# koadman/mauveAligner

Hardware: AMD Instinct MI355X
Metric: aligned Mbp/s (seed+extend+DP) (higher is better)
Workload: dtype u32; 1 GPU; C3: 5 x 5000000 bp synthetic genomes, ~3% divergence, ~50 inversions, seed weight 15, recursive anchoring + gapped DP on; genomes_per_gpu=5, genome_length=5000000, seed_weight=15, parallelism=independent genome sets per GPU (no data-path collective), extend_lcbs=1, max_extension_iters=4

## Files before the change

### mauvealigner_amd/csrc/api.cpp

```cpp
#include "common.hpp"
#include <dlfcn.h>
#include <algorithm>
#include <cstring>

static thread_local std::string g_create_err;

GenomeSet main_genome_set(mauve_ctx *c)
{
    GenomeSet gs;
    gs.buf = &c->genomes; gs.nseq = c->nseq; gs.lens = c->lens; gs.word_off = c->word_off;
    if (c->has_invalid) gs.vmask = &c->base_invalid;
    if (c->has_contigs) gs.cmask = &c->contig_mask;
    if (c->has_invalid || c->has_contigs) gs.mask_off = c->base_mask_off;
    return gs;
}

struct GenomeTails { uint64_t off[MAUVE_MAX_SEQ]; int64_t len[MAUVE_MAX_SEQ]; uint64_t total_words; };
__global__ void genome_tail_fix(uint64_t *__restrict__ words, GenomeTails gt)
{
    const int g = blockIdx.x;
    const int64_t len = gt.len[g];
    const uint64_t data = (uint64_t)((len + 31) / 32);
    uint64_t *w = words + gt.off[g];
    const uint64_t end = (g + 1 == (int)gridDim.x ? gt.total_words + 4 : gt.off[g + 1]) - gt.off[g];
// ... 195 lines not shown
extern "C" {

static hipError_t create_priority_stream(hipStream_t *out)
{
    int least = 0, greatest = 0;
    if (hipDeviceGetStreamPriorityRange(&least, &greatest) != hipSuccess) { (void)hipGetLastError(); return hipStreamCreateWithFlags(out, hipStreamNonBlocking); }
    return hipStreamCreateWithPriority(out, hipStreamNonBlocking, least);
}

int mauve_ctx_create(int device, mauve_ctx **out)
{
    if (!out) return MAUVE_ERR_ARG;
    *out = nullptr;
    int ndev = 0;
    hipError_t e = hipGetDeviceCount(&ndev);
    if (e != hipSuccess || ndev <= 0) {
        g_create_err = std::string("no HIP device available (") + (e != hipSuccess ? hipGetErrorString(e) : "count = 0") +
                       "); libmauve_hip has no CPU fallback";
        return MAUVE_ERR_NOGPU;
    }
    if (device < 0 || device >= ndev) { g_create_err = "device index out of range"; return MAUVE_ERR_ARG; }
    mauve_ctx *c = new (std::nothrow) mauve_ctx();
    if (!c) { g_create_err = "out of host memory"; return MAUVE_ERR_ARG; }
    c->device = device;
    if (const char *sp = getenv("MAUVE_SCHEDULE")) {
        const unsigned f = !strcmp(sp, "spin") ? hipDeviceScheduleSpin : !strcmp(sp, "yield") ? hipDeviceScheduleYield : hipDeviceScheduleBlockingSync;
        (void)hipSetDevice(device); (void)hipSetDeviceFlags(f); (void)hipGetLastError();
    }
    if ((e = hipSetDevice(device)) != hipSuccess || (e = hipStreamCreateWithFlags(&c->stream, hipStreamNonBlocking)) != hipSuccess ||
        (e = create_priority_stream(&c->stream2)) != hipSuccess ||
        (e = hipStreamCreateWithFlags(&c->stream_io, hipStreamNonBlocking)) != hipSuccess ||
        (e = hipEventCreateWithFlags(&c->ev_io_fork, hipEventDisableTiming)) != hipSuccess ||
        (e = hipEventCreateWithFlags(&c->ev_io_done, hipEventDisableTiming)) != hipSuccess ||
        (e = hipEventCreateWithFlags(&c->ev_fork, hipEventDisableTiming)) != hipSuccess ||
        (e = hipEventCreateWithFlags(&c->ev_join, hipEventDisableTiming)) != hipSuccess ||
        (e = hipEventCreate(&c->ev0)) != hipSuccess || (e = hipEventCreate(&c->ev1)) != hipSuccess) {
        g_create_err = std::string("HIP init failed: ") + hipGetErrorString(e);
        delete c;
        return MAUVE_ERR_HIP;
    }
    hipDeviceProp_t prop;
    if (hipGetDeviceProperties(&prop, device) == hipSuccess) {
        snprintf(c->devname, sizeof c->devname, "%s (%s, %d CUs)", prop.name, prop.gcnArchName, prop.multiProcessorCount);
        if (prop.multiProcessorCount > 0) c->cus = prop.multiProcessorCount;
    }
    c->pool = new (std::nothrow) SpinPool(SpinPool::default_threads());
    if (!c->pool) { g_create_err = "out of host memory"; mauve_ctx_destroy(c); return MAUVE_ERR_ARG; }
    *out = c;
    return MAUVE_OK;
}

void mauve_ctx_destroy(mauve_ctx *c)
{
    if (!c) return;
    (void)hipSetDevice(c->device);
    if (c->stream_io) (void)hipStreamSynchronize(c->stream_io);
    if (c->stream2) (void)hipStreamSynchronize(c->stream2);
    if (c->stream) (void)hipStreamSynchronize(c->stream);
    delete c->pool; c->pool = nullptr;
    DevBuf *bufs[] = {&c->genomes, &c->keysA, &c->keysB, &c->valsA, &c->valsB, &c->hist, &c->totals, &c->posmask,
                      &c->hit_mask, &c->hit_pos, &c->hit_seg, &c->base_invalid, &c->contig_mask, &c->node_cmask, &c->run_sum, &c->join_ovf, &c->join_bound, &c->dpf_anch, &c->dpf_work, &c->dpf_tot, &c->ch_len, &c->ch_st, &c->ch_crop, &c->ch_ent, &c->ch_ord, &c->ch_rank, &c->ch_node, &c->ch_graph, &c->ch_cnt, &c->ch_anch, &c->ch_lw, &c->ch_anch2, &c->ext_work, &c->bp_work, &c->dp_sp, &c->hom_cols, &c->sorted_rec_keep, &c->ch_big, &c->gap_work, &c->as_wide, &c->res_narrow, &c->dp_pick, &c->dp_wflags, &c->ch_mw, &c->shard_dev, &c->as_work, &c->as_isl, &c->res_cols, &c->sorted_rec, &c->canon_k1, &c->canon_k2, &c->canon_v1, &c->canon_v2, &c->rec_genomes, &c->rec_seg, &c->rec_vinv, &c->rec_vcm, &c->placed_mask, &c->bb_cols, &c->bb_work, &c->bb_query, &c->cand, &c->mlen, &c->mstart, &c->counters, &c->dp_desc, &c->dp_list, &c->dp_codes, &c->dp_off,
                      &c->dp_prof_cnt, &c->dp_prof_mask, &c->dp_prof2_cnt, &c->dp_prof2_mask, &c->dp_tb, &c->dp_meta,
                      &c->dp_score, &c->dp_cols, &c->dp_rows, &c->rp_wcnt, &c->rp_mult, &c->pf_mums, &c->co_index, &c->co_q, &c->ex_work, &c->ex_bits, &c->ex_sel, &c->ex_mat, &c->ps_work, &c->ps_out, &c->exc_work, &c->exc_tmp, &c->exc_meta, &c->exc_rec, &c->pj_work, &c->pj_cols, &c->pj_src, &c->pj_out, &c->co_truth_index, &c->sc_out, &c->rm_work, &c->rm_res};
    for (DevBuf *b : bufs) b->release();
    coord_index_release(c);
    c->pin_genomes.release(); c->pin_tail.release(); c->pin_ext.release(); c->pin_chain.release(); c->pin_mask.release(); c->pin_bb.release(); c->pin_asm.release(); c->pin_tab.release(); c->pin_cols.release(); c->pin_anch.release(); c->pin_dcols.release(); c->pin_meta.release(); c->pin_seed.release(); c->pin_dp_in.release(); c->shard_pin.release(); c->pin_stage.release();
    if (c->ev0) (void)hipEventDestroy(c->ev0);
    if (c->ev1) (void)hipEventDestroy(c->ev1);
    if (c->ev_fork) (void)hipEventDestroy(c->ev_fork);
    if (c->ev_join) (void)hipEventDestroy(c->ev_join);
    if (c->ev_io_fork) (void)hipEventDestroy(c->ev_io_fork);
    if (c->ev_io_done) (void)hipEventDestroy(c->ev_io_done);
    if (c->stream_io) (void)hipStreamDestroy(c->stream_io);
    if (c->stream2) (void)hipStreamDestroy(c->stream2);
    if (c->stream) (void)hipStreamDestroy(c->stream);
    delete c;
}

const char *mauve_last_error(const mauve_ctx *c) { return c ? c->err.c_str() : g_create_err.c_str(); }

int mauve_device_name(const mauve_ctx *c, char *buf, size_t buflen)
{
    if (!c || !buf || !buflen) return MAUVE_ERR_ARG;
    snprintf(buf, buflen, "%s", c->devname);
    return MAUVE_OK;
}

int mauve_synchronize(mauve_ctx *c)
{
    if (!c) return MAUVE_ERR_ARG;
    HIPCHK(c, hipStreamSynchronize(c->stream));
    return MAUVE_OK;
}

int mauve_set_shard(mauve_ctx *c, int rank, int world, mauve_allgather_fn fn, void *user)
{
    if (!c) return MAUVE_ERR_ARG;
    c->shard_comm = nullptr; c->shard_stat = mauve_shard_stats{0, 0, 0, 0.0};
    if (world <= 1 || !fn) { c->shard_rank = 0; c->shard_world = 1; c->shard_fn = nullptr; c->shard_user = nullptr; c->shard_on = false; return MAUVE_OK; }
    if (rank < 0 || rank >= world) { c->err = "set_shard: rank outside the world"; return MAUVE_ERR_ARG; }
    c->shard_rank = rank; c->shard_world = world; c->shard_fn = fn; c->shard_user = user; c->shard_on = true;
    return MAUVE_OK;
}

int mauve_set_shard_rccl(mauve_ctx *c, int rank, int world, void *nccl_comm)
// ... 332 lines not shown
```

### mauvealigner_amd/csrc/common.hpp

```cpp
#pragma once
#include <hip/hip_runtime.h>
#include <cstdint>
#include <cstdio>
#include <string>
#include <vector>
#include <functional>
#include "workers.hpp"
#include "host_chain.hpp"
#include "backbone_host.hpp"
#include <chrono>
#include <algorithm>
#include <cstring>

#include "../../include/mauve_hip.h"

#define HIPCHK(ctx, call)                                                                         \
    do {                                                                                          \
        hipError_t e__ = (call);                                                                  \
        if (e__ != hipSuccess) {                                                                  \
            (ctx)->err = std::string(#call) + ": " + hipGetErrorString(e__) + " (" __FILE__ ":" + \
                         std::to_string(__LINE__) + ")";                                          \
            return MAUVE_ERR_HIP;                                                                 \
        }                                                                                         \
    } while (0)
// ... 123 lines not shown
    const int32_t *dv_len = nullptr, *dv_st = nullptr, *dv_lcb = nullptr;
    bool lw_from_host = false;
    int64_t mums_kept = -1;
    mauve_params p{};
    int N = 0; uint32_t full = 0;
    int64_t sum = 0, nm = 0, nl = 0, n_dp = 0, code_total = 0, n_anchor = 0, anchor_cols = 0;
    double t0 = 0, t_dp0 = 0;
    std::vector<MatchVec> chains;
    std::vector<GapRef> gaps;
    std::vector<DpSeqDesc> desc;
    std::vector<int64_t> dcol_off, dscore;
    MatchVec m;
    std::vector<int64_t> match_lcb;
    std::vector<int64_t> match_weight;
    std::vector<Item> items;
    void count_anchors() { for (const MatchVec &ch : chains) { n_anchor += (int64_t)ch.size(); for (size_t i = 0; i < ch.size(); i++) anchor_cols += ch.len(i); } }
    void reset()
    {
        open = false; anchor_table_done = false; dev_tail = false; dv_len = dv_st = dv_lcb = nullptr; lw_from_host = false; mums_kept = -1; p = mauve_params(); N = 0; full = 0;
        sum = nm = nl = n_dp = code_total = n_anchor = anchor_cols = 0; t0 = t_dp0 = 0;
        gaps.clear(); desc.clear(); dcol_off.clear(); dscore.clear();
        match_lcb.clear(); match_weight.clear(); items.clear();
    }
};

struct CoordDev;
struct mauve_ctx {
    int device = 0;
    hipStream_t stream = nullptr;
    hipStream_t stream2 = nullptr;
    hipEvent_t ev_fork = nullptr, ev_join = nullptr;
    hipStream_t stream_io = nullptr;
    hipEvent_t ev_io_fork = nullptr, ev_io_done = nullptr;
    struct TablePrefetch {
        int32_t *mum_length = nullptr, *mum_start = nullptr, *anchor_length = nullptr, *anchor_start = nullptr, *anchor_lcb = nullptr;
        int64_t mum_cap = 0, anchor_cap = 0;
        bool armed = false;
        bool live = false;
        bool inflight = false;
        bool got_mums = false, got_anchors = false;
    } pf;
    DevBuf pf_mums;
    std::string err;
    char devname[256] = {0};
    int cus = 256;

    int nseq = 0;
    std::vector<int64_t> lens;
    std::vector<uint64_t> word_off;
    std::vector<const uint64_t *> host_packed;
    PinnedBuf pin_genomes;
    PinnedBuf pin_tail;
    bool host_copy_valid = false;
    size_t total_words = 0;
    DevBuf genomes;
    DevBuf base_invalid, contig_mask, node_cmask;
    bool has_invalid = false, has_contigs = false;
    std::vector<uint64_t> h_invalid, h_contig, base_mask_off;

    DevBuf keysA, keysB, valsA, valsB, hist, totals, posmask, hit_mask, hit_pos, hit_seg, cand, mlen, mstart, counters;
    DevBuf sorted_rec;
    DevBuf canon_k1, canon_k2, canon_v1, canon_v2;
    DevBuf join_bound;
    DevBuf join_ovf;
    DevBuf ch_len, ch_st, ch_crop, ch_ent, ch_ord, ch_rank, ch_node, ch_graph, ch_cnt;
    DevBuf gap_work;
// ... 157 lines not shown
int refuse_past_2g(mauve_ctx *c, const char *what);
int seedpass_run(mauve_ctx *ctx, const GenomeSet &gs, uint64_t pattern, int mode, uint64_t mask, int extend,
                 const uint32_t *seg_dev, uint32_t nseg, int64_t *n_matches);
int seedpass_enumerate(mauve_ctx *ctx, const GenomeSet &gs, int seq, uint64_t pattern, EnumRequest &q);
int seedpass_from_hits(mauve_ctx *ctx, const GenomeSet &gs, uint64_t pattern, const HostHits &hits, int extend, int64_t *n_matches);
int seedpass_sorted_list(mauve_ctx *ctx, const GenomeSet &gs, int seq, uint64_t pattern, std::vector<uint64_t> *keys,
                         std::vector<uint32_t> *vals, int *weight);

int sort_pairs_u32(mauve_ctx *ctx, uint32_t n, int key_bits, uint32_t **keys_io, uint32_t **vals_io, uint32_t *keys_alt, uint32_t *vals_alt,
                   int timer_id);
int sort_pairs_u32_batch(mauve_ctx *ctx, uint32_t S, uint32_t n, size_t seg_stride, int key_bits, uint32_t **keys_io, uint32_t **vals_io,
                         uint32_t *keys_alt, uint32_t *vals_alt, int timer_id);
int sort_pairs_u64(mauve_ctx *ctx, uint32_t n, int key_bits, uint64_t **keys_io, uint32_t **vals_io, uint64_t *keys_alt, uint32_t *vals_alt,
                   int timer_id);
int seed_finish(mauve_ctx *ctx, const GenomeSet &gs, const SeedRequest &rq, uint32_t ncand, bool on_host, double &trace_t0);
bool seed_trace_on();
uint32_t canon_device_min();
inline void seed_trace(mauve_ctx *ctx, const char *label, double &t0)
{
    if (!seed_trace_on()) return;
    (void)hipStreamSynchronize(ctx->stream);
    const double t = now_ms();
    fprintf(stderr, "[trace] %-22s +%.3f ms\n", label, t - t0);
    t0 = t;
}
inline int seed_counters(mauve_ctx *ctx, size_t bytes, const uint32_t **words)
{
    HIPCHK(ctx, ctx->pin_seed.ensure(64));
    HIPCHK(ctx, hipMemcpyAsync(ctx->pin_seed.p, ctx->counters.p, bytes, hipMemcpyDeviceToHost, ctx->stream));
    HIPCHK(ctx, hipStreamSynchronize(ctx->stream));
    *words = ctx->pin_seed.as<uint32_t>();
    return MAUVE_OK;
}
int chain_device(mauve_ctx *c, int N, int64_t min_weight, bool collinear, MatchVec &m, std::vector<int64_t> &match_lcb, int64_t &n_lcb, const mauve_scoring *sp_scoring = nullptr);
struct ChainGraphHost { uint32_t na, K; int64_t *weight; uint32_t *orient; int32_t *prev, *next; int32_t *final_stage; int32_t *final_dev; };
int chain_device_graph(mauve_ctx *c, int N, int64_t maxlen, const uint32_t *seg0, uint32_t nseg, ChainGraphHost *G, bool graph_to_host = true, const mauve_scoring *sp_scoring = nullptr);
int chain_device_gaps_compact(mauve_ctx *c, int N, int64_t maxlen, const uint32_t *seg0_dev, uint32_t nseg, const int32_t **hl_out, const int32_t **hs_out,
                              const uint32_t **hgap_out, uint32_t *ns_out);
int chain_device_core(mauve_ctx *c, int N, int64_t min_weight, bool collinear, int64_t &n_lcb, const mauve_scoring *sp_scoring = nullptr);
int chain_device_gaps(mauve_ctx *c, int N, int64_t maxlen, const uint32_t *seg0_dev, uint32_t nseg, const int32_t **hl_out, const int32_t **hs_out,
                      std::vector<uint8_t> &survive);
int chain_device_copy_back(mauve_ctx *c, int N, MatchVec &m, std::vector<int64_t> &match_lcb);
int chain_order_device(mauve_ctx *c, int N, int64_t nl, int64_t min_gap, int64_t *na_out, int64_t *n_rec_out);
int extend_lcbs_device(mauve_ctx *c, const mauve_params *p, int w, int64_t lcbw, int N, const int32_t **alen_io, const int32_t **ast_io,
                       const int32_t **alcb_io, int64_t *na_io, int64_t *nl_io, int64_t *n_rec_io, std::vector<int64_t> &lcb_weight);

struct ChainOrders { std::vector<std::vector<uint32_t>> ord; bool sparse = false; };
void host_eliminate_overlaps(MatchVec &m, ChainOrders *orders = nullptr, bool compact = true);
int seed_family_matches(mauve_ctx *c, const GenomeSet &gs, int w, int mode, uint64_t mask, MatchVec &out);
void host_merge_matches(MatchVec &kept, const MatchVec &add);
void host_left_orders(const MatchVec &m, ChainOrders &orders);
void host_lcb_chain(const MatchVec &m, int64_t min_weight, bool collinear, std::vector<int64_t> &match_lcb, int64_t &n_lcb,
                    const ChainOrders *orders = nullptr, const int64_t *match_weight = nullptr);
int match_sp_scores(mauve_ctx *c, const MatchVec &m, const int *gmap, const mauve_scoring *sc, std::vector<int64_t> &out);
int repeat_multiplicity(mauve_ctx *c, uint64_t pattern);
int repeat_matches(mauve_ctx *c, int seq, uint64_t pattern, int64_t min_multi, int64_t max_multi);
int repeat_fetch(mauve_ctx *c, int64_t *length, int64_t *mult, int64_t *start_off, int64_t *starts);
int repeat_begin(mauve_ctx *c, const mauve_params *p, int w, uint64_t pat);
int64_t sp_default_min_weight(int w, int n, const mauve_scoring *sc);
int resolve_seed(mauve_ctx *c, const mauve_params *p, int64_t avg_len, const char *who, int *w, uint64_t *pat);
void seed_matches_to_vec(const mauve_ctx *c, int n, int64_t nm, MatchVec &m);
int host_chain_lcbs(mauve_ctx *c, const mauve_params *p, MatchVec &m, const int *gmap, int64_t lcbw, int64_t minw_sp, std::vector<int64_t> &match_lcb,
                    int64_t &nl, std::vector<int64_t> *match_weight, bool compact, double *t_elim = nullptr);
void result_reset(AlignResult &R);
void restore_cols(AlignResult &R, uint32_t full, SpinPool *pool = nullptr);

// ... 52 lines not shown
```

### mauvealigner_amd/csrc/seed_pass.hip

```cpp
#include "common.hpp"
#include "dev_scan.hpp"
#include "radix_sort.hpp"
#include "seed_dev.hpp"
#include <algorithm>
#include <cstring>
#include <cstdlib>
#include <type_traits>

__device__ __forceinline__ uint32_t seg_of(const uint32_t *__restrict__ segs, uint32_t nseg, uint32_t p)
{
    uint32_t lo = 0, hi = nseg;
    while (hi - lo > 1) { uint32_t mid = (lo + hi) >> 1; if (segs[mid] <= p) lo = mid; else hi = mid; }
    return lo;
}
__device__ __forceinline__ bool window_segment(const uint32_t *__restrict__ seg, uint32_t nseg, int g, uint32_t p, int span, uint32_t *id)
{
    const uint32_t *sg = seg + (size_t)g * (nseg + 1);
    const uint32_t k = *id = seg_of(sg, nseg, p);
    return p + span <= sg[k + 1];
}

template <typename KeyT, bool SEG, typename ValT = uint32_t>
__global__ void __launch_bounds__(256) seed_extract(const uint64_t *__restrict__ packed, GenomeTab tab,
                                                    SeedShape sh, int g, KeyT *__restrict__ keys,
                                                    ValT *__restrict__ vals, uint32_t out_base,
                                                    const uint32_t *__restrict__ seg, uint32_t nseg)
{
    uint32_t n = tab.nwin[g];
    const uint64_t *G = packed + tab.word_off[g];
    for (uint32_t p = blockIdx.x * blockDim.x + threadIdx.x; p < n; p += gridDim.x * blockDim.x) {
        const MerKey m = mer_at<false>(G, p, sh);
        uint64_t key = m.key;
        if (SEG) {
            uint32_t k;
            key = window_segment(seg, nseg, g, p, sh.span, &k) ? (((uint64_t)k << (2 * sh.weight)) | key) : ~0ULL;
        }
// ... 461 lines not shown
    }
    emit[i] = e;
}
struct EmitVal { const uint32_t *e; __device__ int64_t value(uint32_t i) const { return e[i]; } };
struct EnumRuns {
    const uint32_t *cnt; const int64_t *soff; uint32_t n; int64_t *mult, *start_off; int64_t *tot ;
    __device__ uint32_t domain(int) const { return n; }
    __device__ bool flag(uint32_t i, int) const { return cnt[i] != 0; }
    __device__ void each(uint32_t, uint32_t, bool, int) const {}
    __device__ void emit(uint32_t i, uint32_t r, int) const { mult[r] = cnt[i]; start_off[r] = soff[i]; }
    __device__ void total(uint32_t runs, int) const { tot[0] = runs; start_off[runs] = soff[n]; }
};
template <typename KeyT, typename ValT = uint32_t>
__global__ void __launch_bounds__(256) enum_write(const KeyT *__restrict__ keys, const ValT *__restrict__ vals, uint32_t n, int direct_only,
                                                  const uint32_t *__restrict__ emit, const int64_t *__restrict__ soff, uint32_t gpos0,
                                                  int64_t *__restrict__ starts)
{
    const uint32_t i = blockIdx.x * 256u + threadIdx.x;
    if (i >= n || emit[i] == 0) return;
    const KeyT k = keys[i];
    const uint32_t ref = win_strand(vals[i]);
    uint32_t j = i; bool found_rev = false;
    while (j < n && keys[j] == k) { if (win_strand(vals[j]) != ref) found_rev = true; j++; }
    int64_t o = soff[i];
    for (uint32_t t = i; t < j; t++) {
        const bool rv = win_strand(vals[t]) != ref;
        const int64_t p1 = (int64_t)(win_idx(vals[t]) - gpos0) + 1;
        if (direct_only && found_rev) { if (!rv) starts[o++] = p1; }
        else starts[o++] = rv ? -p1 : p1;
    }
}


constexpr int RUNS_ITEMS = 16;
constexpr uint32_t RUNS_TILE = 256u * RUNS_ITEMS, RUNS_HALO = 64 ;
static_assert(RUNS_HALO >= MAUVE_MAX_SEED_SPAN && RUNS_HALO == 64, "mum_runs looks back at most one span, and reads the mask word 64 positions in front of every lane");
static_assert(RUNS_ITEMS <= 32, "one bit per item in the hit / pending / flag words");

__device__ __forceinline__ bool same_diagonal(const uint32_t *__restrict__ rp, const uint32_t *__restrict__ rq, uint32_t m, int a,
                                              int nseq, uint32_t d)
{
    const uint32_t sa = rp[a] >> 31, sq = rq[a] >> 31;
    for (int g = a + 1; g < nseq; g++) {
        if (!(m >> g & 1)) continue;
        const uint32_t vp = rp[g], vq = rq[g];
        const uint32_t o = (vp >> 31) ^ sa;
        if (((vq >> 31) ^ sq) != o) return false;
        const uint32_t pp = vp & 0x7fffffffu, pq = vq & 0x7fffffffu;
        if (!(o ? (pq == pp + d) : (pq + d == pp))) return false;
    }
    return true;
}

template <bool SEG>
__device__ __forceinline__ void mum_runs_body(const GenomeTab &tab, int span, const uint32_t *__restrict__ tmask,
                                              const uint32_t *__restrict__ tpos, uint32_t P, int all,
                                              uint32_t *__restrict__ cand, uint32_t *__restrict__ counters,
                                              const uint32_t *__restrict__ seg, uint32_t nseg, uint32_t p0, uint32_t cand_cap)
{
    __shared__ uint32_t lds[8];
    __shared__ uint32_t s_base;
    __shared__ uint32_t s_mask[RUNS_HALO + RUNS_TILE];
    const uint32_t base = p0 + blockIdx.x * RUNS_TILE;
    const int N = tab.nseq;
    uint32_t flags = 0, cnt = 0;
    uint32_t mm[RUNS_ITEMS];
    uint32_t hits = 0;
// ... 14 lines not shown
        __syncthreads();
        const int lane = threadIdx.x & 63;
        uint32_t dd[RUNS_ITEMS];
        uint32_t pend = 0, any = 0;
#pragma unroll
        for (int it = 0; it < RUNS_ITEMS; it++) {
            dd[it] = 0;
            const uint32_t m = mm[it];
            uint64_t left = __ballot(m != 0);
            if (left == 0) continue;
            const uint32_t p = base + it * 256 + threadIdx.x;
            const int a = m ? __ffs(m) - 1 : 0;
            uint32_t g0 = tab.gpos_off[a];
            if (SEG) { if (m) { const uint32_t *sg = seg + (size_t)a * (nseg + 1); g0 += sg[seg_of(sg, nseg, p - g0)]; } }
            const uint32_t lim = m ? min((uint32_t)span, p - g0) : 0u;
            const uint32_t mprev = s_mask[RUNS_HALO + it * 256 + threadIdx.x - 64];
            uint32_t d = 0;
            while (left) {
                const uint32_t mv = (uint32_t)__builtin_amdgcn_readlane((int32_t)m, __ffsll((unsigned long long)left) - 1);
                const uint64_t Bc = __ballot(m == mv), Bp = __ballot(mprev == mv);
                left &= ~Bc;
                const uint64_t W = lane ? ((Bp >> lane) | (Bc << (64 - lane))) : Bp;
                const uint32_t dist = W ? (uint32_t)__clzll((long long)W) + 1u : 0u;
                d = m == mv ? dist : d;
            }
            const bool pd = d != 0 && d <= lim, cd = m != 0 && !pd;
            dd[it] = pd ? d : 0u;
            pend |= (pd ? 1u : 0u) << it; any |= pd ? m : 0u;
            flags |= (cd ? 1u : 0u) << it; cnt += cd ? 1u : 0u;
        }
        uint32_t sa_bits = 0, sq_bits = 0, bad = 0;
        const uint32_t base_h = base >= RUNS_HALO ? base - RUNS_HALO : 0u;
        const uint32_t *tb = tpos + (size_t)base_h * N;
        constexpr int RB = 8;
#pragma unroll
        for (int i0 = 0; i0 < RUNS_ITEMS; i0 += RB) {
            if (!__any((pend >> i0) & ((1u << RB) - 1u))) continue;
            for (int g = 0; g < N; g++) {
                if (!__any((any >> g) & 1u)) continue;
                uint32_t vp[RB], vq[RB];
#pragma unroll
                for (int i = 0; i < RB; i++) {
                    const int it = i0 + i;
                    const uint32_t po = base - base_h + it * 256 + threadIdx.x;
                    const bool mine = ((pend >> it) & 1u) && ((mm[it] >> g) & 1u);
                    vp[i] = tb[mine ? po * (uint32_t)N + (uint32_t)g : 0u];
                    vq[i] = tb[mine ? (po - dd[it]) * (uint32_t)N + (uint32_t)g : 0u];
                }
#pragma unroll
                for (int i = 0; i < RB; i++) {
                    const int it = i0 + i;
                    const bool mine = ((pend >> it) & 1u) && ((mm[it] >> g) & 1u);
                    const bool first = g == __ffs(mm[it]) - 1;
                    sa_bits |= (mine && first) ? (vp[i] >> 31) << it : 0u; sq_bits |= (mine && first) ? (vq[i] >> 31) << it : 0u;
                    const uint32_t o = (vp[i] >> 31) ^ ((sa_bits >> it) & 1u);
                    const uint32_t pp = vp[i] & 0x7fffffffu, pq = vq[i] & 0x7fffffffu;
                    const bool off = (((vq[i] >> 31) ^ ((sq_bits >> it) & 1u)) != o) || !(o ? (pq == pp + dd[it]) : (pq + dd[it] == pp));
                    bad |= (mine && !first && off) ? 1u << it : 0u;
                }
            }
        }
        const uint32_t again = pend & bad;
#pragma unroll
        for (int it = 0; it < RUNS_ITEMS; it++) {
            if (!((again >> it) & 1u)) continue;
            const uint32_t p = base + it * 256 + threadIdx.x, m = mm[it];
            const int a = __ffs(m) - 1;
// ... 187 lines not shown
                bool a = k >= kmin && k <= kmax && ext_window_clean(M1[0], lane, sh);
                if (masks) a = a && !ext_blocked(comp, nc, sh.span, k);
                const uint64_t A = __ballot(a);
                const int p = walk_round(A, sh.span, done);
                cur += p;
            }
            khi = cur;
        }
        if (lane == 0) mlen[ci] = (int32_t)(khi - klo) + sh.span;
        if (lane < N) {
            int32_t st = 0;
            if (mask >> lane & 1) {
                const ExtComp &C = comp[__popc(mask & ((1u << lane) - 1u))];
                st = C.rev ? (int32_t)(-(C.pos - khi + 1)) : (int32_t)(C.pos + klo + 1);
            }
            mstart[(size_t)ci * N + lane] = st;
        }
        __threadfence_block();
#ifdef MAUVE_EXT_STATS
        st_rounds += st_r; st_right += __builtin_amdgcn_s_memrealtime() - st_c2;
#endif
    }
#ifdef MAUVE_EXT_STATS
    if (lane == 0) {
        const unsigned long long dt = __builtin_amdgcn_s_memrealtime() - st_t0;
        atomicAdd(&g_ext_stats[0], st_rounds); atomicAdd(&g_ext_stats[2], dt); atomicMax(&g_ext_stats[3], dt); atomicAdd(&g_ext_stats[4], 1ULL); atomicMax(&g_ext_stats[5], st_rounds);
        atomicAdd(&g_ext_stats[1], st_setup); atomicAdd(&g_ext_stats[6], st_left); atomicAdd(&g_ext_stats[7], st_right);
    }
#endif
}
bool seed_trace_on() { static const bool v = getenv("MAUVE_TRACE") != nullptr; return v; }
static bool no_tiny() { static const bool v = getenv("MAUVE_NO_TINY") != nullptr; return v; }
static uint32_t list_cap_env() { static const uint32_t v = getenv("MAUVE_LIST_CAP") ? (uint32_t)strtoul(getenv("MAUVE_LIST_CAP"), nullptr, 10) : 0u; return v; }
uint32_t canon_device_min() { static const uint32_t v = getenv("MAUVE_CANON_DEVICE_MIN") ? (uint32_t)atol(getenv("MAUVE_CANON_DEVICE_MIN")) : 16384u; return v; }
bool seedpass_wide(int64_t total_windows)
{
    static const bool force = [] { const char *e = getenv("MAUVE_WIDE_INDEX"); return e && e[0] == '1' && e[1] == 0; }();
    return force || total_windows >= (1LL << 31);
}

bool make_seed_shape(uint64_t pattern, SeedShape *sh)
{
    memset(sh, 0, sizeof *sh);
    int span = mauve_seed_length(pattern), w = mauve_seed_weight(pattern);
    if (span < 1 || span > MAUVE_MAX_SEED_SPAN || w < 1 || w > 31) return false;
    for (int t = 0; t < span; t++)
        if (((pattern >> t) & 1) != ((pattern >> (span - 1 - t)) & 1)) return false;
    if (!(pattern & 1)) return false;
    sh->span = span; sh->weight = w; sh->keymask = (1ULL << (2 * w)) - 1ULL;
    int j = 0, nr = 0;
    for (int t = 0; t < span;) {
        if (!((pattern >> (span - 1 - t)) & 1)) { t++; continue; }
        int t0 = t;
        while (t < span && ((pattern >> (span - 1 - t)) & 1)) t++;
        int len = t - t0;
        if (nr >= 32) return false;
        sh->run_src[nr] = (uint8_t)(2 * t0); sh->run_bits[nr] = (uint8_t)(2 * len); sh->run_dst[nr] = (uint8_t)(2 * j);
        nr++; j += len;
    }
    sh->nruns = nr;
    for (int t = 0; t < span; t++) {
        if (!((pattern >> (span - 1 - t)) & 1)) continue;
        if (2 * t < 64) sh->care_lo |= 3ULL << (2 * t); else sh->care_hi |= 3ULL << (2 * t - 64);
    }
    return true;
}
// ... 40 lines not shown

static int seed_plan(mauve_ctx *ctx, const SeedShape &sh, const GenomeTab &tab, const SeedRequest &rq, uint32_t n, bool masked, bool seg,
                     int key_type_bits, SeedPlan *pl, std::vector<FinderPass> *passes)
{
    pl->seg = seg;
    pl->hash_path = !rq.hits && rq.mode != MAUVE_MODE_PAIRWISE && !rq.out_keys && !rq.enumerate && rq.only_seq < 0 && !(masked && seg);
    pl->segbits = 0;
    if (seg) while (pl->segbits < 32 && (1ull << pl->segbits) <= (uint64_t)rq.nseg) pl->segbits++;
    if (seg && 2 * sh.weight + pl->segbits > 64) { ctx->err = "recursive anchoring: segment id and mer do not fit 64 bits"; return MAUVE_ERR_LIMIT; }
    pl->full_bits = seg ? 2 * sh.weight + pl->segbits : ((masked && rq.only_seq >= 0) ? key_type_bits : 2 * sh.weight);
    pl->tiny = pl->hash_path && !no_tiny() && n <= (uint32_t)TJ_MAX && tab.nseq <= 16 && 2 * sh.weight + pl->segbits <= 32;
    pl->compact = !rq.hits && !pl->tiny && rq.only_seq < 0 && masked && !seg;
    pl->has_invalid = masked && !pl->compact;
    const int N = tab.nseq;
    if (rq.mode == MAUVE_MODE_PAIRWISE) {
        int pi = 0;
        for (int i = 0; i < N; i++) for (int j = i + 1; j < N; j++, pi++)
            if (!ctx->pair_sums_only || !ctx->shard_on || pi % ctx->shard_world == ctx->shard_rank)
                passes->push_back({(1u << i) | (1u << j), (1u << i) | (1u << j), MAUVE_MODE_MEM});
    } else passes->push_back({0xffffffffu, (uint32_t)rq.mask, rq.mode});
    pl->use_summary = rq.mode == MAUVE_MODE_PAIRWISE && !seg && !rq.hits && (passes->size() > 1 || (ctx->pair_sums_only && ctx->shard_on && !passes->empty()));
    return MAUVE_OK;
}

struct SeedState {
    mauve_ctx *ctx; const GenomeSet &gs; const SeedShape &sh; const GenomeTab &tab; const SeedRequest &rq;
    uint32_t P;
    const uint64_t *packed, *vmask, *cmask;
    SeedPlan pl;
    std::vector<FinderPass> passes;
    uint32_t ns = 0;
    int L = 0;
    uint32_t *tmask = nullptr, *tpos = nullptr;
    uint32_t cand_cap = 0;
    uint32_t cand_total = 0;
    bool records_on_host = false;
    double trace_t0 = 0;
};
template <typename KeyT, typename ValT>
struct SeedPass : SeedState {
    KeyT *keys = nullptr; ValT *vals = nullptr;
    bool have_hist0 = false;
    SeedPass(const SeedState &s) : SeedState(s) {}
};

template <typename KeyT, typename ValT>
static int ensure_sort_buffers(mauve_ctx *ctx, uint32_t n)
{
    HIPCHK(ctx, ctx->keysA.ensure((size_t)n * sizeof(KeyT)));
    HIPCHK(ctx, ctx->keysB.ensure((size_t)n * sizeof(KeyT)));
    HIPCHK(ctx, ctx->valsA.ensure((size_t)n * sizeof(ValT)));
    HIPCHK(ctx, ctx->valsB.ensure((size_t)n * sizeof(ValT)));
    return MAUVE_OK;
}

template <typename F>
static void launch_narrow_or_not(const SeedShape &sh, F &&launch)
{
    if (seed_narrow(sh)) launch(std::true_type{});
    else launch(std::false_type{});
}

template <typename KeyT, bool SEG, typename ValT>
static int extract_all(mauve_ctx *ctx, const GenomeSet &gs, const SeedShape &sh, const GenomeTab &tab, uint32_t n, const uint32_t *seg, uint32_t nseg,
                       int hshift, KeyT *keys, ValT *vals)
{
// ... 88 lines not shown
        HIPCHK(ctx, hipMemcpyAsync(q.starts, ctx->sorted_rec.p, (size_t)q.ns * 8, hipMemcpyDeviceToHost, ctx->stream));
        HIPCHK(ctx, hipStreamSynchronize(ctx->stream));
    }
    return MAUVE_OK;
}

template <typename KeyT, typename ValT>
static int export_sorted_list(SeedPass<KeyT, ValT> &ps)
{
    constexpr bool WIDEV = sizeof(ValT) == 8;
    mauve_ctx *ctx = ps.ctx; const uint32_t sorted_n = ps.ns;
    std::vector<uint64_t> *out_keys = ps.rq.out_keys; std::vector<uint32_t> *out_vals = ps.rq.out_vals;
    std::vector<KeyT> hk(sorted_n);
    out_vals->resize(sorted_n);
    std::vector<ValT> hv(WIDEV ? sorted_n : 0);
    HIPCHK(ctx, hipMemcpyAsync(hk.data(), ps.keys, (size_t)sorted_n * sizeof(KeyT), hipMemcpyDeviceToHost, ctx->stream));
    HIPCHK(ctx, hipMemcpyAsync(WIDEV ? (void *)hv.data() : (void *)out_vals->data(), ps.vals, (size_t)sorted_n * sizeof(ValT), hipMemcpyDeviceToHost, ctx->stream));
    HIPCHK(ctx, hipStreamSynchronize(ctx->stream));
    out_keys->resize(sorted_n);
    for (uint32_t i = 0; i < sorted_n; i++) (*out_keys)[i] = (uint64_t)hk[i];
    if (WIDEV) {
        const uint32_t g0 = ps.tab.gpos_off[ps.rq.only_seq];
        for (uint32_t i = 0; i < sorted_n; i++) (*out_vals)[i] = ((uint32_t)hv[i] - g0) | ((uint32_t)((uint64_t)hv[i] >> 63) << 31);
    }
    return MAUVE_OK;
}

static bool cand_overflow(SeedState &st, uint32_t nc)
{
    if (nc > st.cand_cap) st.ctx->err = "seed pass: " + std::to_string(nc) + " candidates for a list of " + std::to_string(st.cand_cap);
    return nc > st.cand_cap;
}

template <bool SEG>
static int launch_runs(SeedState &st)
{
    mauve_ctx *ctx = st.ctx; const uint32_t P = st.P;
    { KernelTimer t(ctx, MAUVE_K_RUNS, P);
      hipLaunchKernelGGL((mum_runs<SEG>), dim3((P + RUNS_TILE - 1) / RUNS_TILE), dim3(256), 0, ctx->stream, st.tab,
                         st.sh.span, st.tmask, st.tpos, P, st.rq.extend ? 0 : 1, ctx->cand.as<uint32_t>(), ctx->counters.as<uint32_t>(), st.rq.seg,
                         st.rq.nseg, st.cand_cap, 0u); }
    HIPCHK(ctx, hipGetLastError());
    return MAUVE_OK;
}

template <bool SEG, bool WIDEV>
static int launch_extend(SeedState &st, uint32_t blocks, uint32_t ncand, int32_t *o_len, int32_t *o_start, const uint32_t *ncand_dev = nullptr,
                         uint32_t *counters_out = nullptr)
{
    mauve_ctx *ctx = st.ctx;
    KernelTimer t(ctx, MAUVE_K_EXTEND, ncand);
    hipLaunchKernelGGL((mum_extend<SEG, WIDEV>), dim3(blocks), dim3(256), 0, ctx->stream, st.packed, st.tab, st.sh, st.tmask, st.tpos, st.P,
                       ctx->cand.as<uint32_t>(), ncand, st.rq.extend, o_len, o_start, st.rq.seg, st.rq.nseg, st.vmask, st.cmask, ncand_dev, counters_out);
    HIPCHK(ctx, hipGetLastError());
#ifdef MAUVE_EXT_STATS
    if (seed_trace_on()) {
        unsigned long long h[8]; hipStreamSynchronize(ctx->stream);
        hipMemcpyFromSymbol(h, HIP_SYMBOL(g_ext_stats), sizeof h); unsigned long long z[8] = {0}; hipMemcpyToSymbol(HIP_SYMBOL(g_ext_stats), z, sizeof z);
        fprintf(stderr, "[trace]   extend stats: %llu rounds, %llu waves, wave time mean %.1f us max %.1f us (setup %.1f, left walk %.1f, right walk %.1f), most rounds of a wave %llu\n", h[0], h[4],
                h[4] ? h[2] / (double)h[4] / 100.0 : 0.0, h[3] / 100.0, h[4] ? h[1] / (double)h[4] / 100.0 : 0.0, h[4] ? h[6] / (double)h[4] / 100.0 : 0.0,
                h[4] ? h[7] / (double)h[4] / 100.0 : 0.0, h[5]);
    }
#endif
    return MAUVE_OK;
}

template <bool SEG, bool WIDEV>
static int extend_candidates(SeedState &st, uint32_t nc, uint32_t max_blocks)
{
    mauve_ctx *ctx = st.ctx; const int N = st.tab.nseq;
    HIPCHK(ctx, ctx->mlen.ensure_keep((size_t)(st.cand_total + nc) * 4 + 4, (size_t)st.cand_total * 4, ctx->stream));
    HIPCHK(ctx, ctx->mstart.ensure_keep((size_t)(st.cand_total + nc) * 4 * N + 4, (size_t)st.cand_total * 4 * N, ctx->stream));
    if (int rc = launch_extend<SEG, WIDEV>(st, std::min<uint32_t>((nc + 3) / 4, max_blocks), nc, ctx->mlen.as<int32_t>() + st.cand_total,
                                           ctx->mstart.as<int32_t>() + (size_t)st.cand_total * N)) return rc;
// ... 124 lines not shown
            HIPCHK(ctx, hipMemcpyAsync(keys + s0, kp, (size_t)cnt * sizeof(KeyT), hipMemcpyDeviceToDevice, ctx->stream));
            HIPCHK(ctx, hipMemcpyAsync(vals + s0, vp, (size_t)cnt * sizeof(ValT), hipMemcpyDeviceToDevice, ctx->stream));
        }
        sl_lo[q] = s0; tot_sl += cnt; sl_pre[q + 1] = (uint32_t)tot_sl;
    }
    if (tot_sl) {
        HIPCHK(ctx, ctx->join_bound.ensure((2 * nsl + 1) * 4));
        HIPCHK(ctx, ctx->pin_seed.ensure(64 + (2 * nsl + 1) * 4));
        uint32_t *hp = reinterpret_cast<uint32_t *>(ctx->pin_seed.as<char>() + 64);
        memcpy(hp, sl_lo.data(), nsl * 4); memcpy(hp + nsl, sl_pre.data(), (nsl + 1) * 4);
        HIPCHK(ctx, hipMemcpyAsync(ctx->join_bound.p, hp, (2 * nsl + 1) * 4, hipMemcpyHostToDevice, ctx->stream));
        KernelTimer t(ctx, MAUVE_K_JOIN, (uint32_t)tot_sl);
        hipLaunchKernelGGL((mum_join_slices<KeyT, SEG, ValT>), dim3((uint32_t)((tot_sl + 255) / 256)), dim3(256), 0, ctx->stream, (const KeyT *)keys, (const ValT *)vals,
                           ctx->join_bound.as<uint32_t>(), ctx->join_bound.as<uint32_t>() + nsl, (uint32_t)nsl, ps.tab, fp.rule, fp.want,
                           fp.consider, ps.tmask, ps.tpos, (int)ps.pl.has_invalid);
        HIPCHK(ctx, hipStreamSynchronize(ctx->stream));
    }
    HIPCHK(ctx, hipGetLastError());
    HIPCHK(ctx, hipMemsetAsync(ctx->counters.p, 0, 64, ctx->stream));
    if (int rc = launch_runs<SEG>(ps)) return rc;
    const uint32_t *cw;
    if (int rc = seed_counters(ctx, 16, &cw)) return rc;
    *nc = cw[1];
    if (seed_trace_on()) fprintf(stderr, "[trace]   join_hash handed back %u range(s)\n", novf);
    return MAUVE_OK;
}

template <typename KeyT, bool SEG, typename ValT>
static int finder_pass(SeedPass<KeyT, ValT> &ps, const FinderPass &fp)
{
    constexpr bool WIDEV = sizeof(ValT) == 8;
    mauve_ctx *ctx = ps.ctx; const uint32_t P = ps.P, ns = ps.ns; const int N = ps.tab.nseq;
    const HostHits *hh = ps.rq.hits;
    HIPCHK(ctx, hipMemsetAsync(ps.tmask, 0, (size_t)P * 4, ctx->stream));
    HIPCHK(ctx, hipMemsetAsync(ctx->counters.p, 0, 64, ctx->stream));
    if (hh) {
        HIPCHK(ctx, ctx->run_sum.ensure((size_t)hh->n * (N + 1) * 4 + 64));
        HIPCHK(ctx, hipMemcpyAsync(ctx->run_sum.p, hh->rec, (size_t)hh->n * (N + 1) * 4, hipMemcpyHostToDevice, ctx->stream));
        if (hh->n) hipLaunchKernelGGL(hits_scatter<WIDEV>, dim3((hh->n + 255) / 256), dim3(256), 0, ctx->stream, ctx->run_sum.as<uint32_t>(), hh->n, N, P, ps.tmask, ps.tpos, ps.tab);
        HIPCHK(ctx, hipStreamSynchronize(ctx->stream));
    } else if (ps.pl.hash_path) {
        const uint32_t nchunk = (ns + HJ_T - 1) / HJ_T;
        HIPCHK(ctx, ctx->join_ovf.ensure((2 + 2 * (size_t)HJ_OVF_CAP) * 4));
        KernelTimer t(ctx, MAUVE_K_JOIN, ns);
        HIPCHK(ctx, ctx->join_bound.ensure(((size_t)nchunk + 2) * 4));
        hipLaunchKernelGGL((join_bounds<KeyT>), dim3((nchunk + 1 + 3) / 4), dim3(256), 0, ctx->stream, ps.keys, ns, ps.L, nchunk,
                           ctx->join_bound.as<uint32_t>());
#define JH_LAUNCH(W) hipLaunchKernelGGL((join_hash<KeyT, W, ValT>), dim3(nchunk), dim3(256), 0, ctx->stream, ps.keys, ps.vals, ns, \
                                           ctx->join_bound.as<uint32_t>(), ps.tab, fp.rule, fp.want, ps.tmask, ps.tpos, ctx->counters.as<uint32_t>() + 8, ctx->join_ovf.as<uint32_t>(), P)
        if (N > 16) JH_LAUNCH(true);
        else JH_LAUNCH(false);
#undef JH_LAUNCH
    } else
    { KernelTimer t(ctx, MAUVE_K_JOIN, ns);
      hipLaunchKernelGGL((mum_join<KeyT, SEG, ValT>), dim3((ns + 255) / 256), dim3(256), 0, ctx->stream, ps.keys, ps.vals, ns, ps.tab, fp.rule,
                         fp.want, fp.consider, ps.tmask, ps.tpos, P, (int)ps.pl.has_invalid); }
    HIPCHK(ctx, hipGetLastError());
    seed_trace(ctx, "join", ps.trace_t0);
    if (int rc = launch_runs<SEG>(ps)) return rc;
    if (ctx->shadow) { std::function<void()> f; f.swap(ctx->shadow); f(); }
    const uint32_t *cw;
    if (int rc = seed_counters(ctx, 48, &cw)) return rc;
    uint32_t nc = cw[1];
    const uint32_t novf = ps.pl.hash_path ? cw[8] : 0u;
    if (ps.pl.hash_path && cw[9]) { ctx->err = "join_hash: anchor out of range (internal error)"; return MAUVE_ERR_HIP; }
    if (novf) if (int rc = join_overflow_slices<KeyT, SEG, ValT>(ps, fp, novf, &nc)) return rc;
    if (cand_overflow(ps, nc)) return MAUVE_ERR_LIMIT;
    seed_trace(ctx, "runs", ps.trace_t0);
    if (seed_trace_on()) fprintf(stderr, "[trace]   %u candidates of %u windows\n", nc, P);
    if (nc == 0) return MAUVE_OK;
    constexpr int EXT_BLOCKS_PER_CU = 12;
    return extend_candidates<SEG, WIDEV>(ps, nc, (uint32_t)(ctx->cus * EXT_BLOCKS_PER_CU));
}

template <typename KeyT, bool SEG, typename ValT>
static int seedpass_stages(const SeedState &st0)
{
    constexpr bool WIDEV = sizeof(ValT) == 8;
    SeedPass<KeyT, ValT> ps(st0);
    mauve_ctx *ctx = ps.ctx; const SeedRequest &rq = ps.rq; const uint32_t P = ps.P; const int N = ps.tab.nseq;
    if (seed_trace_on()) fprintf(stderr, "[trace] seed pass: %u windows, %d-bit keys, %s window index (%d-bit values)\n", P, (int)sizeof(KeyT) * 8,
                                  WIDEV ? "wide" : "narrow", (int)sizeof(ValT) * 8);
    if (int rc = seed_plan(ctx, ps.sh, ps.tab, rq, P, ps.vmask || ps.cmask, SEG, (int)sizeof(KeyT) * 8, &ps.pl, &ps.passes)) return rc;
    if (int rc = extract<KeyT, SEG, ValT>(ps)) return rc;
    if (ps.ns == 0) { if (rq.n_matches) *rq.n_matches = 0; return MAUVE_OK; }
    ps.L = ps.pl.low_bits(ps.ns);
    if (!rq.hits && !ps.pl.tiny)
        if (int rc = sort_pairs<KeyT, ValT>(ctx, ps.ns, ps.pl.full_bits, &ps.keys, &ps.vals, ctx->keysB.as<KeyT>(), ctx->valsB.as<ValT>(), ps.have_hist0, -1, ps.L)) return rc;
    seed_trace(ctx, "sort", ps.trace_t0);
    if (rq.enumerate) return export_enumerator(ps);
    if (rq.out_keys) return export_sorted_list(ps);

    HIPCHK(ctx, ctx->posmask.ensure((size_t)P * 4));
    HIPCHK(ctx, ctx->hit_pos.ensure((size_t)P * 4 * N));
    ps.tmask = ctx->posmask.as<uint32_t>(); ps.tpos = ctx->hit_pos.as<uint32_t>();
    ps.cand_cap = P / 2 + 1;
    HIPCHK(ctx, ctx->cand.ensure((size_t)ps.cand_cap * 4));
    if (list_cap_env()) ps.cand_cap = std::min(ps.cand_cap, list_cap_env());
    ctx->sdh.hl.clear(); ctx->sdh.hs.clear();
    if (ps.pl.tiny) {
        if (int rc = tiny_pass<SEG, WIDEV>(ps, ps.passes[0])) return rc;
    } else if (ps.pl.use_summary) {
        if (int rc = pairwise_passes(ps)) return rc;
    } else {
        for (const FinderPass &fp : ps.passes)
            if (int rc = finder_pass<KeyT, SEG, ValT>(ps, fp)) return rc;
    }
    return seed_finish(ctx, ps.gs, rq, ps.cand_total, ps.records_on_host, ps.trace_t0);
}

static int seedpass_prologue(mauve_ctx *ctx, const GenomeSet &gs, uint64_t pattern, const int *seq, SeedShape *sh, GenomeTab *tab, int64_t *total)
{
    if (!make_seed_shape(pattern, sh)) { ctx->err = "seed pattern must be palindromic, span <= 49, weight <= 31"; return MAUVE_ERR_ARG; }
    if (!seq && gs.nseq < 1) { ctx->err = "no genomes set"; return MAUVE_ERR_STATE; }
    if (seq && (*seq < 0 || *seq >= gs.nseq)) { ctx->err = "sequence index out of range"; return MAUVE_ERR_ARG; }
    return build_tab(ctx, gs, sh->span, tab, total);
}

static void reset_match_list(mauve_ctx *ctx, int64_t *n_matches)
{
    ctx->n_matches = 0; ctx->match_len.clear(); ctx->match_start.clear(); ctx->matches_pending = false;
    ctx->dev_rec_n = -1;
    if (n_matches) *n_matches = 0;
}

static int seedpass_dispatch(mauve_ctx *ctx, const GenomeSet &gs, const SeedShape &sh, const GenomeTab &tab, int64_t total, const SeedRequest &rq)
{
    SeedState st{ctx, gs, sh, tab, rq, (uint32_t)total, gs.buf->as<uint64_t>(), gs.vmask ? gs.vmask->as<uint64_t>() : nullptr,
// ... 169 lines not shown
```

Before: 10200 Mbp/s.

## Restrict hit table to anchor genome range and overlap speculative extension with count readback

Narrows the hit-mask clear and the mum_runs launch to the window range of the anchoring genome instead of all windows. For single-pass extend runs, it copies the counters to the host on the I/O stream and speculatively launches extension with a capped candidate count while that copy is in flight. If the real count fits the cap, the second extension is skipped. RUNS_ITEMS is also halved to launch more, smaller tiles. The cost is extra buffer allocation and an extra stream dependency, and the speculative extension does wasted work if it overflows.

```diff
diff --git a/mauvealigner_amd/csrc/api.cpp b/mauvealigner_amd/csrc/api.cpp
--- a/mauvealigner_amd/csrc/api.cpp
+++ b/mauvealigner_amd/csrc/api.cpp
@@ -251,6 +251,8 @@
         (e = hipStreamCreateWithFlags(&c->stream_io, hipStreamNonBlocking)) != hipSuccess ||
         (e = hipEventCreateWithFlags(&c->ev_io_fork, hipEventDisableTiming)) != hipSuccess ||
         (e = hipEventCreateWithFlags(&c->ev_io_done, hipEventDisableTiming)) != hipSuccess ||
+        (e = hipEventCreateWithFlags(&c->ev_seed_fork, hipEventDisableTiming)) != hipSuccess ||
+        (e = hipEventCreateWithFlags(&c->ev_seed_done, hipEventDisableTiming)) != hipSuccess ||
         (e = hipEventCreateWithFlags(&c->ev_fork, hipEventDisableTiming)) != hipSuccess ||
         (e = hipEventCreateWithFlags(&c->ev_join, hipEventDisableTiming)) != hipSuccess ||
         (e = hipEventCreate(&c->ev0)) != hipSuccess || (e = hipEventCreate(&c->ev1)) != hipSuccess) {
@@ -290,6 +292,8 @@
     if (c->ev_join) (void)hipEventDestroy(c->ev_join);
     if (c->ev_io_fork) (void)hipEventDestroy(c->ev_io_fork);
     if (c->ev_io_done) (void)hipEventDestroy(c->ev_io_done);
+    if (c->ev_seed_fork) (void)hipEventDestroy(c->ev_seed_fork);
+    if (c->ev_seed_done) (void)hipEventDestroy(c->ev_seed_done);
     if (c->stream_io) (void)hipStreamDestroy(c->stream_io);
     if (c->stream2) (void)hipStreamDestroy(c->stream2);
     if (c->stream) (void)hipStreamDestroy(c->stream);
diff --git a/mauvealigner_amd/csrc/common.hpp b/mauvealigner_amd/csrc/common.hpp
--- a/mauvealigner_amd/csrc/common.hpp
+++ b/mauvealigner_amd/csrc/common.hpp
@@ -179,6 +179,7 @@
     hipEvent_t ev_fork = nullptr, ev_join = nullptr;
     hipStream_t stream_io = nullptr;
     hipEvent_t ev_io_fork = nullptr, ev_io_done = nullptr;
+    hipEvent_t ev_seed_fork = nullptr, ev_seed_done = nullptr;
     struct TablePrefetch {
         int32_t *mum_length = nullptr, *mum_start = nullptr, *anchor_length = nullptr, *anchor_start = nullptr, *anchor_lcb = nullptr;
         int64_t mum_cap = 0, anchor_cap = 0;
@@ -402,6 +403,23 @@
     *words = ctx->pin_seed.as<uint32_t>();
     return MAUVE_OK;
 }
+inline int side_counters_begin(mauve_ctx *ctx, size_t bytes)
+{
+    HIPCHK(ctx, ctx->pin_seed.ensure(64));
+    HIPCHK(ctx, hipEventRecord(ctx->ev_seed_fork, ctx->stream));
+    hipError_t e = hipStreamWaitEvent(ctx->stream_io, ctx->ev_seed_fork, 0);
+    if (e == hipSuccess) e = hipMemcpyAsync(ctx->pin_seed.p, ctx->counters.p, bytes, hipMemcpyDeviceToHost, ctx->stream_io);
+    if (e == hipSuccess) e = hipEventRecord(ctx->ev_seed_done, ctx->stream_io);
+    if (e != hipSuccess) (void)hipStreamSynchronize(ctx->stream_io);
+    HIPCHK(ctx, e);
+    return MAUVE_OK;
+}
+inline int side_counters_wait(mauve_ctx *ctx, const uint32_t **words)
+{
+    HIPCHK(ctx, hipEventSynchronize(ctx->ev_seed_done));
+    *words = ctx->pin_seed.as<uint32_t>();
+    return MAUVE_OK;
+}
 int chain_device(mauve_ctx *c, int N, int64_t min_weight, bool collinear, MatchVec &m, std::vector<int64_t> &match_lcb, int64_t &n_lcb, const mauve_scoring *sp_scoring = nullptr);
 struct ChainGraphHost { uint32_t na, K; int64_t *weight; uint32_t *orient; int32_t *prev, *next; int32_t *final_stage; int32_t *final_dev; };
 int chain_device_graph(mauve_ctx *c, int N, int64_t maxlen, const uint32_t *seg0, uint32_t nseg, ChainGraphHost *G, bool graph_to_host = true, const mauve_scoring *sp_scoring = nullptr);
diff --git a/mauvealigner_amd/csrc/seed_pass.hip b/mauvealigner_amd/csrc/seed_pass.hip
--- a/mauvealigner_amd/csrc/seed_pass.hip
+++ b/mauvealigner_amd/csrc/seed_pass.hip
@@ -2,6 +2,7 @@
 #include "dev_scan.hpp"
 #include "radix_sort.hpp"
 #include "seed_dev.hpp"
+#include "seed_range.hpp"
 #include <algorithm>
 #include <cstring>
 #include <cstdlib>
@@ -529,7 +530,7 @@
 }
 
 
-constexpr int RUNS_ITEMS = 16;
+constexpr int RUNS_ITEMS = 8;
 constexpr uint32_t RUNS_TILE = 256u * RUNS_ITEMS, RUNS_HALO = 64 ;
 static_assert(RUNS_HALO >= MAUVE_MAX_SEED_SPAN && RUNS_HALO == 64, "mum_runs looks back at most one span, and reads the mask word 64 positions in front of every lane");
 static_assert(RUNS_ITEMS <= 32, "one bit per item in the hit / pending / flag words");
@@ -610,7 +611,7 @@
         uint32_t sa_bits = 0, sq_bits = 0, bad = 0;
         const uint32_t base_h = base >= RUNS_HALO ? base - RUNS_HALO : 0u;
         const uint32_t *tb = tpos + (size_t)base_h * N;
-        constexpr int RB = 8;
+        constexpr int RB = RUNS_ITEMS < 8 ? RUNS_ITEMS : 8;
 #pragma unroll
         for (int i0 = 0; i0 < RUNS_ITEMS; i0 += RB) {
             if (!__any((pend >> i0) & ((1u << RB) - 1u))) continue;
@@ -864,6 +865,12 @@
 bool seed_trace_on() { static const bool v = getenv("MAUVE_TRACE") != nullptr; return v; }
 static bool no_tiny() { static const bool v = getenv("MAUVE_NO_TINY") != nullptr; return v; }
 static uint32_t list_cap_env() { static const uint32_t v = getenv("MAUVE_LIST_CAP") ? (uint32_t)strtoul(getenv("MAUVE_LIST_CAP"), nullptr, 10) : 0u; return v; }
+constexpr uint32_t SPEC_CAP = 4u << 20;
+static uint32_t spec_cap()
+{
+    static const uint32_t v = [] { const char *e = getenv("MAUVE_SPEC_CAP"); const uint32_t x = e ? (uint32_t)strtoul(e, nullptr, 10) : 0u; return x ? std::min(x, SPEC_CAP) : SPEC_CAP; }();
+    return v;
+}
 uint32_t canon_device_min() { static const uint32_t v = getenv("MAUVE_CANON_DEVICE_MIN") ? (uint32_t)atol(getenv("MAUVE_CANON_DEVICE_MIN")) : 16384u; return v; }
 bool seedpass_wide(int64_t total_windows)
 {
@@ -970,6 +977,7 @@
     uint32_t ns = 0;
     int L = 0;
     uint32_t *tmask = nullptr, *tpos = nullptr;
+    AnchorRange ar{0, 0};
     uint32_t cand_cap = 0;
     uint32_t cand_total = 0;
     bool records_on_host = false;
@@ -1124,14 +1132,22 @@
     return nc > st.cand_cap;
 }
 
+static int clear_hit_range(SeedState &st)
+{
+    const uint32_t lo = st.ar.lo >= RUNS_HALO ? st.ar.lo - RUNS_HALO : 0u, hi = st.ar.hi;
+    if (hi > lo) HIPCHK(st.ctx, hipMemsetAsync(st.tmask + lo, 0, (size_t)(hi - lo) * 4, st.ctx->stream));
+    return MAUVE_OK;
+}
+
 template <bool SEG>
 static int launch_runs(SeedState &st)
 {
-    mauve_ctx *ctx = st.ctx; const uint32_t P = st.P;
-    { KernelTimer t(ctx, MAUVE_K_RUNS, P);
-      hipLaunchKernelGGL((mum_runs<SEG>), dim3((P + RUNS_TILE - 1) / RUNS_TILE), dim3(256), 0, ctx->stream, st.tab,
-                         st.sh.span, st.tmask, st.tpos, P, st.rq.extend ? 0 : 1, ctx->cand.as<uint32_t>(), ctx->counters.as<uint32_t>(), st.rq.seg,
-                         st.rq.nseg, st.cand_cap, 0u); }
+    mauve_ctx *ctx = st.ctx; const uint32_t lo = st.ar.lo, hi = st.ar.hi;
+    if (hi <= lo) return MAUVE_OK;
+    { KernelTimer t(ctx, MAUVE_K_RUNS, hi - lo);
+      hipLaunchKernelGGL((mum_runs<SEG>), dim3((hi - lo + RUNS_TILE - 1) / RUNS_TILE), dim3(256), 0, ctx->stream, st.tab,
+                         st.sh.span, st.tmask, st.tpos, hi, st.rq.extend ? 0 : 1, ctx->cand.as<uint32_t>(), ctx->counters.as<uint32_t>(), st.rq.seg,
+                         st.rq.nseg, st.cand_cap, lo); }
     HIPCHK(ctx, hipGetLastError());
     return MAUVE_OK;
 }
@@ -1322,7 +1338,8 @@
     constexpr bool WIDEV = sizeof(ValT) == 8;
     mauve_ctx *ctx = ps.ctx; const uint32_t P = ps.P, ns = ps.ns; const int N = ps.tab.nseq;
     const HostHits *hh = ps.rq.hits;
-    HIPCHK(ctx, hipMemsetAsync(ps.tmask, 0, (size_t)P * 4, ctx->stream));
+    ps.ar = (hh || SEG) ? AnchorRange{0u, P} : seed_anchor_range(fp.want, N, ps.tab.gpos_off, P);
+    if (int rc = clear_hit_range(ps)) return rc;
     HIPCHK(ctx, hipMemsetAsync(ctx->counters.p, 0, 64, ctx->stream));
     if (hh) {
         HIPCHK(ctx, ctx->run_sum.ensure((size_t)hh->n * (N + 1) * 4 + 64));
@@ -1348,9 +1365,25 @@
     HIPCHK(ctx, hipGetLastError());
     seed_trace(ctx, "join", ps.trace_t0);
     if (int rc = launch_runs<SEG>(ps)) return rc;
-    if (ctx->shadow) { std::function<void()> f; f.swap(ctx->shadow); f(); }
+    constexpr int EXT_BLOCKS_PER_CU = 12;
+    const uint32_t ext_blocks = (uint32_t)(ctx->cus * EXT_BLOCKS_PER_CU);
+    const bool beside = ps.passes.size() == 1 && ps.cand_total == 0 && ps.rq.extend && !WIDEV && !hh && ps.ar.hi > ps.ar.lo;
+    const uint32_t spec = std::min(ps.cand_cap, spec_cap());
+    if (seed_trace_on()) fprintf(stderr, "[trace]   hit table [%u, %u) of %u windows (%s), extension %s\n", ps.ar.lo, ps.ar.hi, P,
+                                 hh ? "host hits" : ps.pl.hash_path ? "join_hash" : "mum_join", beside ? "beside the count" : "behind the count");
     const uint32_t *cw;
-    if (int rc = seed_counters(ctx, 48, &cw)) return rc;
+    if (beside) {
+        HIPCHK(ctx, ctx->mlen.ensure((size_t)spec * 4 + 4));
+        HIPCHK(ctx, ctx->mstart.ensure((size_t)spec * 4 * N + 4));
+        if (int rc = side_counters_begin(ctx, 48)) return rc;
+        const int rc_ext = launch_extend<SEG, WIDEV>(ps, std::min<uint32_t>((spec + 3) / 4, ext_blocks), spec, ctx->mlen.as<int32_t>(), ctx->mstart.as<int32_t>(), ctx->counters.as<uint32_t>() + 1);
+        if (ctx->shadow) { std::function<void()> f; f.swap(ctx->shadow); f(); }
+        if (int rc = side_counters_wait(ctx, &cw)) return rc;
+        if (rc_ext) return rc_ext;
+    } else {
+        if (ctx->shadow) { std::function<void()> f; f.swap(ctx->shadow); f(); }
+        if (int rc = seed_counters(ctx, 48, &cw)) return rc;
+    }
     uint32_t nc = cw[1];
     const uint32_t novf = ps.pl.hash_path ? cw[8] : 0u;
     if (ps.pl.hash_path && cw[9]) { ctx->err = "join_hash: anchor out of range (internal error)"; return MAUVE_ERR_HIP; }
@@ -1359,8 +1392,12 @@
     seed_trace(ctx, "runs", ps.trace_t0);
     if (seed_trace_on()) fprintf(stderr, "[trace]   %u candidates of %u windows\n", nc, P);
     if (nc == 0) return MAUVE_OK;
-    constexpr int EXT_BLOCKS_PER_CU = 12;
-    return extend_candidates<SEG, WIDEV>(ps, nc, (uint32_t)(ctx->cus * EXT_BLOCKS_PER_CU));
+    if (beside && !novf && nc <= spec) {
+        ps.cand_total = nc;
+        seed_trace(ctx, "extend (beside the count)", ps.trace_t0);
+        return MAUVE_OK;
+    }
+    return extend_candidates<SEG, WIDEV>(ps, nc, ext_blocks);
 }
 
 template <typename KeyT, bool SEG, typename ValT>
@@ -1384,6 +1421,7 @@
     HIPCHK(ctx, ctx->posmask.ensure((size_t)P * 4));
     HIPCHK(ctx, ctx->hit_pos.ensure((size_t)P * 4 * N));
     ps.tmask = ctx->posmask.as<uint32_t>(); ps.tpos = ctx->hit_pos.as<uint32_t>();
+    ps.ar = {0u, P};
     ps.cand_cap = P / 2 + 1;
     HIPCHK(ctx, ctx->cand.ensure((size_t)ps.cand_cap * 4));
     if (list_cap_env()) ps.cand_cap = std::min(ps.cand_cap, list_cap_env());
diff --git a/mauvealigner_amd/csrc/seed_range.hpp b/mauvealigner_amd/csrc/seed_range.hpp
--- /dev/null
+++ b/mauvealigner_amd/csrc/seed_range.hpp
@@ -0,0 +1,12 @@
+#pragma once
+#include <algorithm>
+#include <cstdint>
+
+struct AnchorRange { uint32_t lo, hi; };
+inline AnchorRange seed_anchor_range(uint32_t want, int N, const uint32_t *gpos_off, uint32_t P)
+{
+    const uint32_t all = N >= 32 ? 0xffffffffu : ((1u << N) - 1u);
+    if (N < 2 || (want & ~all)) return {0u, P};
+    if (want) { const int a = __builtin_ctz(want); return {std::min(gpos_off[a], P), std::min(gpos_off[a + 1], P)}; }
+    return {0u, std::min(gpos_off[N - 1], P)};
+}
```

Result: no change. 10350 Mbp/s (median of 3 runs) (+1.5%).
